# stevenlsw/reart

Measured on NVIDIA B200. Metric: skinned_chamfer_fwd_bwd_directed_point_pairs_per_s, higher is better.
Workload: dtype f32

## Files before the change

### include/reart_b200.h

```cpp
#ifndef REART_B200_H_
#define REART_B200_H_

#include <stdint.h>

#ifdef __cplusplus
extern "C" {
#endif

#if defined(__GNUC__)
#define REART_API __attribute__((visibility("default")))
#else
#define REART_API
#endif

#define REART_OK 0
#define REART_ERR_INVALID_ARG (-1)
#define REART_ERR_WORKSPACE (-2)
#define REART_ERR_LAUNCH (-3)
#define REART_ERR_UNSUPPORTED (-4)

REART_API const char* reart_version(void);
REART_API const char* reart_error_string(int code);
REART_API const char* reart_last_cuda_error(void);

// ... 42 lines not shown
REART_API int reart_skinned_chamfer_fwd_bwd_culled(const float* cano, const float* W, const float* R, const float* tr,
                                                   const float* tgt, const float* tgt_packed, int64_t T, int64_t N,
                                                   int64_t M, int64_t P, float* skinned, double* loss, float* gW,
                                                   float* gR, float* gtr, float* g_skinned, int compute_grad,
                                                   float* d_fwd, int64_t* i_fwd, float* d_bwd, int64_t* i_bwd,
                                                   int32_t* nn_rows, int32_t* nn_cols, uint64_t* cull_stats,
                                                   void* workspace, int64_t workspace_bytes, void* stream);
REART_API int reart_skinned_chamfer_fwd_bwd_ordered(const float* cano, const float* W, const float* R, const float* tr,
                                                    const float* tgt, const float* tgt_search, const float* tgt_search_packed,
                                                    int64_t T, int64_t N, int64_t M, int64_t P, const int32_t* row_order,
                                                    const int32_t* row_inv, const int32_t* tgt_order, const int32_t* tgt_inv,
                                                    float* skinned, double* loss, float* gW, float* gR, float* gtr,
                                                    float* g_skinned, int compute_grad, float* d_fwd, int64_t* i_fwd,
                                                    float* d_bwd, int64_t* i_bwd, int32_t* nn_rows, int32_t* nn_cols,
                                                    uint64_t* stats, void* workspace, int64_t workspace_bytes, void* stream);
REART_API int reart_skinned_chamfer_fwd_bwd_fused(const float* cano, const float* hot, const float* W, const float* R,
                                                  const float* tr, const float* tgt, const float* tgt_packed, int64_t T,
                                                  int64_t N, int64_t M, int64_t P, float* skinned, double* loss, float* gW,
                                                  float* gR, float* gtr, float* g_skinned, int compute_grad,
                                                  void* workspace, int64_t workspace_bytes, void* stream);


REART_API int reart_segmlp_fwd(const float* x, const float* w0, const float* b0, const float* w2, int64_t N, int64_t H,
                               int64_t P, float* logits, void* stream);
REART_API int reart_segmlp_bwd(const float* x, const float* w0, const float* b0, const float* w2, const float* glogits,
                               int64_t N, int64_t H, int64_t P, float* gw0, float* gb0, float* gw2, void* stream);
REART_API int reart_gumbel_st_fwd(const float* logits, const float* expo, const float* tau, int64_t N, int64_t P,
                                  float* W, float* ysoft, void* stream);
REART_API int reart_gumbel_st_bwd(const float* ysoft, const float* tau, const float* gW, int64_t N, int64_t P,
                                  float* glogits, void* stream);
// ... 124 lines not shown
```

### reart_b200/_lib.py

```python
from __future__ import annotations

import ctypes
import os

import torch

_HERE = os.path.dirname(os.path.abspath(__file__))
SO_PATH = os.path.join(_HERE, "csrc", "libreart_b200.so")

_c_i64 = ctypes.c_int64
_c_int = ctypes.c_int
_vp = ctypes.c_void_p

SIGNATURES = {
    "reart_version": (ctypes.c_char_p, []),
    "reart_error_string": (ctypes.c_char_p, [_c_int]),
    "reart_last_cuda_error": (ctypes.c_char_p, []),
    "reart_knn1_workspace_bytes": (_c_i64, [_c_i64, _c_i64, _c_i64]),
    "reart_knn1_fwd": (_c_int, [_vp, _vp, _c_i64, _c_i64, _c_i64, _vp, _vp, _vp, _c_i64, _vp]),
    "reart_chamfer_workspace_bytes": (_c_i64, [_c_i64, _c_i64, _c_i64]),
    "reart_chamfer_bidir_fwd": (_c_int, [_vp, _vp, _c_i64, _c_i64, _c_i64, _vp, _vp, _vp, _vp, _vp, _c_i64, _vp]),
    "reart_chamfer_sym_search": (_c_int, [_vp, _vp, _c_i64, _c_i64, _c_i64, _vp, _vp, ctypes.POINTER(ctypes.c_int32), _c_int,
                                          _vp]),
    "reart_knn1_bwd": (_c_int, [_vp, _vp, _vp, _vp, _c_i64, _c_i64, _c_i64, _vp, _vp, _vp]),
# ... 1 lines not shown
    "reart_packed_bytes": (_c_i64, [_c_i64, _c_i64]),
    "reart_pack_cloud": (_c_int, [_vp, _c_i64, _c_i64, _vp, _vp]),
    "reart_skin_fwd": (_c_int, [_vp, _vp, _vp, _vp, _c_i64, _c_i64, _c_i64, _vp, _vp]),
    "reart_skin_bwd_workspace_bytes": (_c_i64, [_c_i64, _c_i64, _c_i64]),
    "reart_skin_bwd": (_c_int, [_vp, _vp, _vp, _vp, _vp, _c_i64, _c_i64, _c_i64, _vp, _vp, _vp, _vp, _c_i64, _vp]),
    "reart_energy_workspace_bytes": (_c_i64, [_c_i64, _c_i64, _c_i64]),
    "reart_skinned_chamfer_fwd_bwd": (_c_int, [_vp, _vp, _vp, _vp, _vp, _vp, _c_i64, _c_i64, _c_i64, _c_i64, _vp, _vp,
                                               _vp, _vp, _vp, _vp, _c_int, _vp, _c_i64, _vp]),
    "reart_skinned_chamfer_fwd_bwd_ex": (_c_int, [_vp, _vp, _vp, _vp, _vp, _vp, _c_i64, _c_i64, _c_i64, _c_i64, _vp, _vp,
                                                  _vp, _vp, _vp, _vp, _c_int, _vp, _vp, _vp, _vp, _vp, _c_i64, _vp]),
    "reart_skinned_chamfer_fwd_bwd_culled": (_c_int, [_vp, _vp, _vp, _vp, _vp, _vp, _c_i64, _c_i64, _c_i64, _c_i64, _vp, _vp,
                                                      _vp, _vp, _vp, _vp, _c_int, _vp, _vp, _vp, _vp, _vp, _vp, _vp, _vp, _c_i64,
                                                      _vp]),
    "reart_skinned_chamfer_fwd_bwd_ordered": (_c_int, [_vp] * 7 + [_c_i64] * 4 + [_vp] * 10 + [_c_int] + [_vp] * 8 +
                                              [_c_i64, _vp]),
    "reart_segmlp_fwd": (_c_int, [_vp, _vp, _vp, _vp, _c_i64, _c_i64, _c_i64, _vp, _vp]),
    "reart_segmlp_bwd": (_c_int, [_vp, _vp, _vp, _vp, _vp, _c_i64, _c_i64, _c_i64, _vp, _vp, _vp, _vp]),
    "reart_gumbel_st_fwd": (_c_int, [_vp, _vp, _vp, _c_i64, _c_i64, _vp, _vp, _vp]),
    "reart_gumbel_st_bwd": (_c_int, [_vp, _vp, _vp, _c_i64, _c_i64, _vp, _vp]),
    "reart_rot6d_fwd": (_c_int, [_vp, _c_i64, _vp, _vp]),
    "reart_rot6d_bwd": (_c_int, [_vp, _vp, _c_i64, _vp, _vp]),
    "reart_screw_to_transform_fwd": (_c_int, [_vp, _vp, _vp, _vp, _c_i64, _vp, _vp]),
    "reart_screw_to_transform_bwd": (_c_int, [_vp, _vp, _vp, _vp, _vp, _c_i64, _vp, _vp, _vp, _vp, _vp]),
    "reart_fk_fwd": (_c_int, [_vp, _vp, _vp, _vp, _vp, _vp, _vp, _vp, _c_i64, _c_i64, _vp, _vp]),
    "reart_fk_bwd": (_c_int, [_vp, _vp, _vp, _vp, _vp, _vp, _vp, _vp, _c_i64, _c_i64, _vp, _vp, _vp, _vp, _vp, _vp,
                              _vp, _vp]),
    "reart_knn": (_c_int, [_vp, _vp, _c_i64, _c_i64, _c_i64, _c_int, _vp, _vp, _vp]),
    "reart_knn_sq": (_c_int, [_vp, _vp, _c_i64, _c_i64, _c_i64, _c_int, _vp, _vp, _vp]),
    "reart_knn3_blend": (_c_int, [_vp, _vp, _vp, _vp, _c_i64, _c_i64, _vp, _vp, _vp]),
    "reart_flow_refs_sorted_bytes": (_c_i64, [_c_i64, _c_i64]),
# ... 97 lines not shown
```

### reart_b200/csrc/capi.cu

```cuda
#include "../../include/reart_b200.h"
#include "common.cuh"
#include "kernels.h"

using namespace reart;

namespace {

constexpr int64_t kAlign = 256;
inline int64_t align_up(int64_t v) { return round_up(v, kAlign); }
inline bool fits_int(int64_t v) { return v >= 0 && v <= 0x7fffffff; }

#define REART_ENTRY() (void)cudaGetLastError()

struct Carver {
    char* base;
    int64_t off;
    int64_t cap;
    bool ok;
    Carver(void* p, int64_t bytes) : base(static_cast<char*>(p)), off(0), cap(bytes), ok(p != nullptr || bytes == 0) {}
    template <typename T>
    T* take(int64_t count) {
        const int64_t bytes = align_up(count * (int64_t)sizeof(T));
        if (!ok || off + bytes > cap) { ok = false; return nullptr; }
        T* r = reinterpret_cast<T*>(base + off);
// ... 205 lines not shown
                                            compute_grad, nullptr, nullptr, nullptr, nullptr, workspace, workspace_bytes, stream_);
}

int reart_skinned_chamfer_fwd_bwd_ex(const float* cano, const float* W, const float* R, const float* tr, const float* tgt,
                                     const float* tgt_packed, int64_t T, int64_t N, int64_t M, int64_t P, float* skinned,
                                     double* loss, float* gW, float* gR, float* gtr, float* g_skinned, int compute_grad,
                                     float* d_fwd, int64_t* i_fwd, float* d_bwd, int64_t* i_bwd, void* workspace,
                                     int64_t workspace_bytes, void* stream_) {
    REART_ENTRY();
    return reart_skinned_chamfer_fwd_bwd_culled(cano, W, R, tr, tgt, tgt_packed, T, N, M, P, skinned, loss, gW, gR, gtr, g_skinned,
                                                compute_grad, d_fwd, i_fwd, d_bwd, i_bwd, nullptr, nullptr, nullptr, workspace,
                                                workspace_bytes, stream_);
}

struct SearchOrder {
    const int32_t* row_order; const int32_t* row_inv; const int32_t* tgt_order; const int32_t* tgt_inv;
    const float* tgt_search;
};

static int energy_pipeline(const float* cano, const float* W, const float* hot, const float* R, const float* tr,
                           const float* tgt, const float* tgt_packed, int64_t T, int64_t N, int64_t M, int64_t P,
                           float* skinned, double* loss, float* gW, float* gR, float* gtr, float* g_skinned, int compute_grad,
                           float* d_fwd, int64_t* i_fwd, float* d_bwd, int64_t* i_bwd, int32_t* nn_rows, int32_t* nn_cols,
                           uint64_t* cull_stats, void* workspace, int64_t workspace_bytes, void* stream_,
                           const SearchOrder* order = nullptr);

int reart_skinned_chamfer_fwd_bwd_culled(const float* cano, const float* W, const float* R, const float* tr,
                                         const float* tgt, const float* tgt_packed, int64_t T, int64_t N, int64_t M,
                                         int64_t P, float* skinned, double* loss, float* gW, float* gR, float* gtr,
                                         float* g_skinned, int compute_grad, float* d_fwd, int64_t* i_fwd, float* d_bwd,
                                         int64_t* i_bwd, int32_t* nn_rows, int32_t* nn_cols, uint64_t* cull_stats,
                                         void* workspace, int64_t workspace_bytes, void* stream_) {
// ... 1 lines not shown
    return energy_pipeline(cano, W, nullptr, R, tr, tgt, tgt_packed, T, N, M, P, skinned, loss, gW, gR, gtr, g_skinned,
                           compute_grad, d_fwd, i_fwd, d_bwd, i_bwd, nn_rows, nn_cols, cull_stats, workspace, workspace_bytes,
                           stream_);
}

int reart_skinned_chamfer_fwd_bwd_ordered(const float* cano, const float* W, const float* R, const float* tr,
                                          const float* tgt, const float* tgt_search, const float* tgt_search_packed,
                                          int64_t T, int64_t N, int64_t M, int64_t P, const int32_t* row_order,
                                          const int32_t* row_inv, const int32_t* tgt_order, const int32_t* tgt_inv,
                                          float* skinned, double* loss, float* gW, float* gR, float* gtr, float* g_skinned,
                                          int compute_grad, float* d_fwd, int64_t* i_fwd, float* d_bwd, int64_t* i_bwd,
                                          int32_t* nn_rows, int32_t* nn_cols, uint64_t* stats, void* workspace,
                                          int64_t workspace_bytes, void* stream_) {
    REART_ENTRY();
    if (!tgt_search || !row_order || !row_inv || !tgt_order || !tgt_inv || !nn_rows || !nn_cols) return REART_ERR_INVALID_ARG;
    const SearchOrder order = {row_order, row_inv, tgt_order, tgt_inv, tgt_search};
    return energy_pipeline(cano, W, nullptr, R, tr, tgt, tgt_search_packed, T, N, M, P, skinned, loss, gW, gR, gtr, g_skinned,
                           compute_grad, d_fwd, i_fwd, d_bwd, i_bwd, nn_rows, nn_cols, stats, workspace, workspace_bytes,
                           stream_, &order);
}

int reart_skinned_chamfer_fwd_bwd_fused(const float* cano, const float* hot, const float* W, const float* R,
                                        const float* tr, const float* tgt, const float* tgt_packed, int64_t T, int64_t N,
                                        int64_t M, int64_t P, float* skinned, double* loss, float* gW, float* gR,
                                        float* gtr, float* g_skinned, int compute_grad, void* workspace,
                                        int64_t workspace_bytes, void* stream_) {
    REART_ENTRY();
    if (!hot || (reinterpret_cast<uintptr_t>(hot) & 15) || (reinterpret_cast<uintptr_t>(cano) & 15) ||
        (reinterpret_cast<uintptr_t>(skinned) & 15))
        return REART_ERR_INVALID_ARG;
    return energy_pipeline(cano, W, hot, R, tr, tgt, tgt_packed, T, N, M, P, skinned, loss, gW, gR, gtr, g_skinned, compute_grad,
// ... 32 lines not shown
    if (!ws.ok) return REART_ERR_WORKSPACE;
    long long* acc = reinterpret_cast<long long*>(zero);
    unsigned* ticket = reinterpret_cast<unsigned*>(zero + T * N * 24);
    unsigned* col_bound = ticket + 1;
    if (cudaMemsetAsync(zero, 0, (size_t)zero_bytes, stream) != cudaSuccess) return REART_ERR_LAUNCH;
    int rc = kOk;
    SymParams sp = {};
    sp.a = skinned; sp.b_packed = tgt_packed; sp.keys_a = ka; sp.keys_b = kb;
    sp.B = (int)T; sp.na = (int)N; sp.nb = (int)M; sp.nb_pad = (int)padded_points(M);
    sp.col_bound = col_bound;
    sp.keys_one_allocation = 1;
    if (hot) {
        if (cull) return REART_ERR_INVALID_ARG;
        sp.sk_cano = cano; sp.sk_hot = hot; sp.sk_R = R; sp.sk_tr = tr; sp.sk_P = (int)P; sp.sk_npad = (int)n_pad_sorted;
        sp.sk_out = skinned; sp.sk_sorted = psrc; sp.sk_perm = perm; sp.sk_xq = xq;
    } else {
        rc = launch_skin_fwd_sorted(cano, W, R, tr, T, N, P, skinned, psrc, perm, xq, n_pad_sorted, stream,
                                    order ? order->row_order : nullptr, skinned_search);
        if (rc) return rc;
    }
    if (order) {
        sp.a = skinned_search;
        sp.tie_a = tie; sp.tie_b = tie + T * N;
    }
    if (cull) {
        CullParams cp = {};
        cp.a = sp.a; cp.b = order ? order->tgt_search : tgt; cp.nn_rows = nn_rows; cp.nn_cols = nn_cols;
        cp.B = (int)T; cp.na = (int)N; cp.nb = (int)M; cp.nb_pad = (int)padded_points(M);
        cp.colbox = colbox; cp.rowbound = rowbound;
        cp.coarse = (N >= 8192 && M >= 8192 && N <= 800000 && M <= 800000) ? 1 : 0;
        rc = launch_cull_bounds(cp, stream);
        if (rc) return rc;
        sp.cull = 1; sp.colbox = colbox; sp.rowbound = rowbound;
        sp.cull_stats = reinterpret_cast<unsigned long long*>(cull_stats);
    }
    rc = launch_chamfer_sym(sp, stream);
    if (rc) return rc;
    EnergyParams ep = {};
    ep.src = skinned; ep.tgt = tgt; ep.src_packed = psrc; ep.tgt_packed = tgt_packed; ep.keys_a = ka; ep.keys_b = kb;
    ep.B = (int)T; ep.N = (int)N; ep.M = (int)M; ep.n_pad = (int)n_pad_sorted; ep.m_pad = (int)padded_points(M);
    ep.row_chunk_pts = kChunk; ep.col_chunk_pts = sp.col_chunk_pts; ep.gscale = 1.0f; ep.g_src = gs; ep.loss = loss;
    if (sp.col_chunk_pts != 256) return REART_ERR_UNSUPPORTED;
    ep.d_fwd = d_fwd; ep.i_fwd = i_fwd; ep.d_bwd = d_bwd; ep.i_bwd = i_bwd;
    ep.nn_rows = nn_rows; ep.nn_cols = nn_cols;
    ep.src_perm = perm; ep.src_xq = xq; ep.acc = acc; ep.col_bound = col_bound; ep.partials = partials; ep.ticket = ticket;
    if (order) {
        ep.row_order = order->row_order; ep.row_inv = order->row_inv; ep.tgt_order = order->tgt_order; ep.tgt_inv = order->tgt_inv;
        ep.tie_a = sp.tie_a; ep.tie_b = sp.tie_b;
        ep.ties = cull_stats ? reinterpret_cast<unsigned long long*>(cull_stats) + 2 : nullptr;
    }
    rc = launch_energy_bwd(ep, stream);
    if (rc || !compute_grad) return rc;
    return launch_skin_bwd(cano, W, R, tr, gs, T, N, P, gW, gR, gtr, bwd_partials, stream);
}

int reart_segmlp_fwd(const float* x, const float* w0, const float* b0, const float* w2, int64_t N, int64_t H, int64_t P,
                     float* logits, void* stream_) {
    REART_ENTRY();
    if (N < 0 || H <= 0 || P <= 0) return REART_ERR_INVALID_ARG;
    if (N == 0) return REART_OK;
    if (!x || !w0 || !b0 || !w2 || !logits) return REART_ERR_INVALID_ARG;
    return launch_segmlp(x, w0, b0, w2, nullptr, N, H, P, logits, nullptr, nullptr, nullptr,
// ... 389 lines not shown
```

### reart_b200/csrc/cull.cu

```cuda
#include "common.cuh"
#include "kernels.h"
#include <algorithm>

namespace reart {

constexpr int kCullRowChunk = 256;
constexpr int kCullSeeds = 4;
constexpr int kCoarse = 256;

__device__ __forceinline__ float coarse_upper_bound(const float* __restrict__ pts, int n, const float* __restrict__ s_rep,
                                                    int nrep, float qx, float qy, float qz) {
    float a0 = INFINITY, a1 = INFINITY;
    int r0 = 0, r1 = 0;
    for (int r = 0; r < nrep; ++r) {
        const float d = sqdist_scalar(qx, qy, qz, s_rep[3 * r], s_rep[3 * r + 1], s_rep[3 * r + 2]);
        if (d < a0) { a1 = a0; r1 = r0; a0 = d; r0 = r; }
        else if (d < a1) { a1 = d; r1 = r; }
    }
    float ub = a0;
    float b0 = INFINITY;
    int c0 = -1;
#pragma unroll 1
    for (int h = 0; h < 2; ++h) {
        const int r = h ? r1 : r0;
// ... 48 lines not shown
    }
    unsigned bits = 0u;
    if (i < p.na) {
        float ub = INFINITY;
        const float* a = p.a + ((int64_t)b * p.na + i) * 3;
        const float ax = a[0], ay = a[1], az = a[2];
        if (p.coarse) {
            ub = coarse_upper_bound(p.b + (int64_t)b * p.nb * 3, p.nb, s_rep, nrep, ax, ay, az);
            if (!(ub >= 0.f)) ub = INFINITY;
        }
        if (p.nn_rows) {
            int jprev = -2;
#pragma unroll
            for (int d = -kCullSeeds; d <= kCullSeeds; ++d) {
                const int in = min(max(i + d, 0), p.na - 1);
                const int j = p.nn_rows[(int64_t)b * p.na + in];
                if (j == jprev) continue;
                jprev = j;
                if (j >= 0 && j < p.nb) {
                    const float* t = p.b + ((int64_t)b * p.nb + j) * 3;
                    const float c = sqdist_scalar(ax, ay, az, t[0], t[1], t[2]);
                    if (c < ub) ub = c;
                }
            }
        }
        bits = __float_as_uint(ub);
    }
    bits = __reduce_max_sync(0xffffffffu, bits);
    if ((threadIdx.x & 31) == 0) s_w[threadIdx.x >> 5] = bits;
    __syncthreads();
    if (threadIdx.x == 0) {
        unsigned m = 0u;
#pragma unroll
        for (int w = 0; w < kCullRowChunk / 32; ++w) m = max(m, s_w[w]);
        p.rowbound[(int64_t)b * row_chunks + rc] = __uint_as_float(m);
// ... 15 lines not shown
    float lx = INFINITY, ly = INFINITY, lz = INFINITY, hx = -INFINITY, hy = -INFINITY, hz = -INFINITY;
    unsigned bits = 0u;
    if (j < p.nb) {
        const float* t = p.b + ((int64_t)b * p.nb + j) * 3;
        const float x = t[0], y = t[1], z = t[2];
        lx = hx = x; ly = hy = y; lz = hz = z;
        float ub = INFINITY;
        if (p.coarse) {
            ub = coarse_upper_bound(p.a + (int64_t)b * p.na * 3, p.na, s_rep, nrep, x, y, z);
            if (!(ub >= 0.f)) ub = INFINITY;
        }
        if (p.nn_cols) {
#pragma unroll
            for (int d = -kCullSeeds; d <= kCullSeeds; ++d) {
                const int jn = min(max(j + d, 0), p.nb - 1);
                const int i0 = p.nn_cols[(int64_t)b * p.nb + jn];
                if (i0 < 0 || i0 >= p.na) continue;
#pragma unroll
                for (int e = -1; e <= 1; ++e) {
                    if (d != 0 && e != 0) continue;
                    const int i = min(max(i0 + e, 0), p.na - 1);
                    const float* a = p.a + ((int64_t)b * p.na + i) * 3;
                    const float c = sqdist_scalar(a[0], a[1], a[2], x, y, z);
                    if (c < ub) ub = c;
                }
            }
        }
        bits = __float_as_uint(ub);
    }
#pragma unroll
    for (int o = 16; o > 0; o >>= 1) {
        lx = fminf(lx, __shfl_xor_sync(0xffffffffu, lx, o)); ly = fminf(ly, __shfl_xor_sync(0xffffffffu, ly, o));
// ... 29 lines not shown
```

### reart_b200/csrc/energy.cu

```cuda
#include "common.cuh"
#include "kernels.h"
#include <algorithm>

namespace reart {

constexpr int kEnergyThreads = 256;

__device__ __forceinline__ double block_sum(double local, double* sh) {
#pragma unroll
    for (int o = 16; o > 0; o >>= 1) local += __shfl_xor_sync(0xffffffffu, local, o);
    if ((threadIdx.x & 31) == 0) sh[threadIdx.x >> 5] = local;
    __syncthreads();
    double s = 0.0;
    if (threadIdx.x == 0) {
#pragma unroll
        for (int w = 0; w < kEnergyThreads / 32; ++w) s += sh[w];
    }
    return s;
}

__device__ __forceinline__ int warp_lowest_match(const float* __restrict__ pts, int n, float qx, float qy, float qz, float d) {
    const int lane = threadIdx.x & 31;
    constexpr int kPer = 16;
    for (int j0 = 0; j0 < n; j0 += 32 * kPer) {
// ... 43 lines not shown
        int i = 0;
        bool flagged = false;
        if (valid) {
            b = f / p.M;
            s = ORDERED ? b * p.M + p.tgt_inv[f] : f;
            const u64 key = p.keys_b[s];
            dmin = __uint_as_float((unsigned)(key >> 32));
            const float* a = p.tgt + f * 3;
            ax = a[0]; ay = a[1]; az = a[2];
            flagged = ORDERED && p.tie_b[s] == (unsigned)(key >> 32);
            if (!flagged) {
                i = rescan_sorted_chunk_q(p.src_packed + b * (int64_t)p.n_pad * 3, p.src_perm + b * (int64_t)p.n_pad,
                                          p.src_xq + b * (int64_t)(p.n_pad / kSortedChunk) * kQuantiles,
                                          (unsigned)(key & 0xffffffffu), ax, ay, az, dmin);
                if (i >= p.N) i = 0;
                if (ORDERED) i = p.row_order[i];
            }
        }
        if (ORDERED) resolve_flagged(flagged, p.src, p.N, ax, ay, az, dmin, b, i, p.ties);
        if (!valid) continue;
        const float* t = p.src + (b * p.N + i) * 3;
        unsigned long long* go = reinterpret_cast<unsigned long long*>(p.acc) + (b * p.N + i) * 3;
        atomicAdd(go + 0, (unsigned long long)__float2ll_rn(-g2 * (ax - t[0]) * scale));
        atomicAdd(go + 1, (unsigned long long)__float2ll_rn(-g2 * (ay - t[1]) * scale));
        atomicAdd(go + 2, (unsigned long long)__float2ll_rn(-g2 * (az - t[2]) * scale));
        local += (double)dmin;
        if (p.d_bwd) p.d_bwd[f] = dmin;
        if (p.i_bwd) p.i_bwd[f] = i;
        if (p.nn_cols) p.nn_cols[s] = ORDERED ? p.row_inv[i] : i;
    }
    const double s = block_sum(local, sh);
    if (threadIdx.x == 0) p.partials[blockIdx.x] = s;
}

template <bool ORDERED>
__global__ void __launch_bounds__(kEnergyThreads) energy_rows_kernel(const EnergyParams p, int col_blocks) {
    __shared__ double sh[kEnergyThreads / 32];
    __shared__ bool last;
    const int64_t total = (int64_t)p.B * p.N;
    const float g2 = 2.0f * p.gscale;
    const float inv = ldexpf(1.0f, -fixed_point_exponent(*p.col_bound, fabsf(g2), p.M));
    double local = 0.0;
    const int lane = threadIdx.x & 31;
    for (int64_t e0 = blockIdx.x * (int64_t)blockDim.x + (threadIdx.x - lane); e0 < total; e0 += (int64_t)gridDim.x * blockDim.x) {
        const int64_t e = e0 + lane;
        const bool valid = e < total;
        int64_t b = 0, s = 0;
        float dmin = 0.f, ax = 0.f, ay = 0.f, az = 0.f;
        int j = 0;
        bool flagged = false;
        if (valid) {
            b = e / p.N;
            s = ORDERED ? b * p.N + p.row_inv[e - b * p.N] : e;
            const u64 key = p.keys_a[s];
            dmin = __uint_as_float((unsigned)(key >> 32));
            const float* a = p.src + e * 3;
            ax = a[0]; ay = a[1]; az = a[2];
            flagged = ORDERED && p.tie_a[s] == (unsigned)(key >> 32);
            if (!flagged) {
                j = rescan_chunk32(p.tgt_packed + b * (int64_t)p.m_pad * 3, (unsigned)(key & 0xffffffffu), ax, ay, az, dmin);
                if (j >= p.M) j = 0;
                if (ORDERED) j = p.tgt_order[b * p.M + j];
            }
        }
        if (ORDERED) resolve_flagged(flagged, p.tgt, p.M, ax, ay, az, dmin, b, j, p.ties);
        if (!valid) continue;
        const long long* ac = p.acc + e * 3;
        const long long c0 = ac[0], c1 = ac[1], c2 = ac[2];
        const float* t = p.tgt + (b * p.M + j) * 3;
        p.g_src[e * 3 + 0] = g2 * (ax - t[0]) + (float)c0 * inv;
        p.g_src[e * 3 + 1] = g2 * (ay - t[1]) + (float)c1 * inv;
        p.g_src[e * 3 + 2] = g2 * (az - t[2]) + (float)c2 * inv;
        local += (double)dmin;
        if (p.d_fwd) p.d_fwd[e] = dmin;
        if (p.i_fwd) p.i_fwd[e] = j;
        if (p.nn_rows) p.nn_rows[s] = ORDERED ? p.tgt_inv[b * p.M + j] : j;
    }
    const double s = block_sum(local, sh);
    if (threadIdx.x == 0) {
        p.partials[col_blocks + blockIdx.x] = s;
        __threadfence();
        last = atomicAdd(p.ticket, 1u) == gridDim.x - 1;
    }
    __syncthreads();
    if (last) {
        __shared__ double tree[kEnergyThreads];
        __threadfence();
        const volatile double* v = p.partials;
        const int n = col_blocks + (int)gridDim.x;
        double tot = 0.0;
        for (int k = threadIdx.x; k < n; k += kEnergyThreads) tot += v[k];
// ... 41 lines not shown
```

### reart_b200/csrc/kernels.h

```cpp
#pragma once
#include <cuda_runtime.h>
#include <stdint.h>

namespace reart {

struct KnnDir {
    const float* q;
    const float* tpacked;
    unsigned long long* keys;
    float* out_dists;
    int64_t* out_idx;
    int nq;
    int nt;
    int nt_pad;
    int qblocks;
    int splits;
    int keys_preset;
    int chunk_pts;
    const unsigned char* perm;
    const float* xq;
};

struct KnnParams {
    KnnDir dir[2];
// ... 24 lines not shown
    const float* sk_cano;
    const float* sk_hot;
    const float* sk_R;
    const float* sk_tr;
    int sk_P, sk_npad;
    float* sk_out;
    float* sk_sorted;
    unsigned char* sk_perm;
    float* sk_xq;
};
struct CullParams {
    const float* a;
    const float* b;
    const int32_t* nn_rows;
    const int32_t* nn_cols;
    int B, na, nb, nb_pad;
    float* colbox;
    float* rowbound;
    int coarse;
};
int launch_cull_bounds(const CullParams& p, cudaStream_t stream);

int launch_pack_cloud(const float* pts, float* packed, int64_t B, int64_t P, cudaStream_t stream);
int launch_pack_cloud_sorted(const float* pts, float* packed, unsigned char* perm, float* xq, int64_t B, int64_t P,
                             int64_t n_pad, cudaStream_t stream);
int launch_knn1_search(KnnParams& p, cudaStream_t stream);
int launch_knn1_finalize(const KnnParams& p, cudaStream_t stream);
int launch_chamfer_sym(SymParams& p, cudaStream_t stream);

int launch_knn1_bwd(const float* p1, const float* p2, const int64_t* idx, const float* grad_dists, int64_t B,
                    int64_t P1, int64_t P2, float* grad_p1, float* grad_p2, int accumulate, cudaStream_t stream);

int launch_chamfer_bidir_bwd(const float* src, const float* tgt, const int64_t* i_fwd, const int64_t* i_bwd,
                             const float* g_fwd, const float* g_bwd, int64_t B, int64_t N, int64_t M, float* grad_src,
                             float* grad_tgt, cudaStream_t stream);

int launch_skin_fwd(const float* cano, const float* W, const float* R, const float* tr, int64_t T, int64_t N, int64_t P,
                    float* out, float* out_packed, cudaStream_t stream);
int launch_skin_fwd_sorted(const float* cano, const float* W, const float* R, const float* tr, int64_t T, int64_t N,
                           int64_t P, float* out, float* out_packed, unsigned char* perm, float* xq, int64_t n_pad,
                           cudaStream_t stream, const int32_t* order = nullptr, float* out_search = nullptr);
int64_t skin_bwd_workspace_floats(int64_t T, int64_t N, int64_t P);
int launch_skin_bwd(const float* cano, const float* W, const float* R, const float* tr, const float* g, int64_t T,
                    int64_t N, int64_t P, float* gW, float* gR, float* gtr, float* partials, cudaStream_t stream);

int launch_rot6d_fwd(const float* d6, int64_t B, float* R, cudaStream_t stream);
int launch_rot6d_bwd(const float* d6, const float* gR, int64_t B, float* gd6, cudaStream_t stream);
int launch_screw_fwd(const float* l, const float* m, const float* theta, const float* d, int64_t B, float* M,
                     cudaStream_t stream);
int launch_screw_bwd(const float* l, const float* m, const float* theta, const float* d, const float* gM, int64_t B,
                     float* gl, float* gm, float* gtheta, float* gd, cudaStream_t stream);

struct FkParams {
// ... 22 lines not shown
    const unsigned long long* keys_b;
    int B, N, M, n_pad, m_pad;
    int row_chunk_pts, col_chunk_pts;
    float gscale;
    float* g_src;
    double* loss;
    long long* acc;
    const unsigned* col_bound;
    double* partials;
    unsigned* ticket;
    int32_t* nn_rows; int32_t* nn_cols;
    float* d_fwd; int64_t* i_fwd;
    float* d_bwd; int64_t* i_bwd;
    const int32_t* row_order;
    const int32_t* row_inv;
    const int32_t* tgt_order;
    const int32_t* tgt_inv;
    const unsigned* tie_a;
    const unsigned* tie_b;
    unsigned long long* ties;
};
int energy_max_blocks();
int launch_energy_bwd(const EnergyParams& p, cudaStream_t stream);

int launch_knn(const float* ref, const float* query, int64_t B, int64_t n, int64_t m, int k, float* dist, int64_t* idx,
               int squared, cudaStream_t stream);
int64_t flow_refs_sorted_floats(int64_t total_refs, int64_t T);
int launch_flow_refs_sort(const float* ref_cat, const int64_t* ref_off, int64_t T, int64_t max_refs, float* sorted,
                          int64_t* sorted_off, cudaStream_t stream);
int launch_knn3_blend_sorted(const float* query, const float* sorted, const int64_t* sorted_off, const float* flow_cat,
// ... 133 lines not shown
```

### reart_b200/engine.py

```python
from __future__ import annotations

import ctypes
import math
from typing import Optional

import torch
import torch.nn.functional as F

from . import _lib, ops
from ._lib import check, ptr, stream_ptr
from .dist import (DistContext, GradBucket, OneShotAllReduce, flow_pairs_for_rank, flow_window_plan, halo_from_previous_rank,
                   make_small_all_reduce, shard_bounds)
from .model import BaseModel, KinematicModel


class _EngineBase:
    def __init__(self, cano: torch.Tensor, frames: torch.Tensor, ctx: Optional[DistContext], use_graph: bool, flow_ref,
                 cano_idx: int, lambda_flow: float, robust_flow: bool):
        self.ctx = ctx or DistContext()
        self.use_graph = use_graph
        self._graphs = {}
        self.iteration = 0
        if frames.shape[0] < self.ctx.world_size:
            raise ValueError(f"{frames.shape[0]} frames cannot be sharded over {self.ctx.world_size} ranks: every rank must "
                             "own at least one frame (an empty shard would skip the step's collectives)")
        lo, hi = self.ctx.frames(frames.shape[0])
        self.frame_range = (lo, hi)
        self.total_frames = int(frames.shape[0])
        self.cano = cano.float().contiguous()
        self.frames = frames[lo:hi].float().contiguous()
        self.pairs_per_step_local = 2 * (hi - lo) * self.cano.shape[0] * self.frames.shape[1]
        if flow_ref is not None and (flow_ref.T != self.total_frames or not 0 <= cano_idx <= self.total_frames):
            raise ValueError(f"the flow reference needs one set per pair of the complete sequence ({self.total_frames}) and "
                             f"0 <= cano_idx <= {self.total_frames}")
        self.flow_ref, self.cano_idx, self.lambda_flow, self.robust_flow = flow_ref, cano_idx, lambda_flow, robust_flow
        self.tau = torch.ones((), device=self.cano.device)
        self.native = self.cull = self.search_culled = False
        self.sink = self.assign = self.optimizer = self.bucket = None
        self._nat = self._ingest_src = self._cur_variant = None

    def _run_iteration(self):
        src = self._ingest_src
        if src is not None:
            cano_src, frames_src = src
            self.cano.copy_(cano_src)
            self.frames.copy_(frames_src)
            ops.pack_cloud(self.frames, out=self.frames_packed)
            if self.search_culled:
                torch.gather(self.frames, 1, self._search_gather, out=self.frames_search)
                ops.pack_cloud(self.frames_search, out=self.frames_search_packed)
        if self.native:
            return self._run_iteration_native()
# ... 148 lines not shown
        finally:
            self._ingest_src = None

    def _after_replay(self, variant):
        if variant[2]:
            self.assign.have_assignment = True

    def _setup_search(self, search: str, can_order: bool, why: str):
        if search not in ("auto", "brute", "culled"):
            raise ValueError("search must be 'auto', 'brute' or 'culled'")
        if search == "culled" and not can_order:
            raise ValueError(why)
        self.search_culled = can_order and (search == "culled" or (
            search == "auto" and min(self.cano.shape[0], self.frames.shape[1]) >= SEARCH_CULLED_MIN_POINTS))
        self.search_order_rows = self.search_order_tgt = None
        if self.search_culled:
            dev = self.cano.device
            self.search_order_rows = ops.search_order(self.cano[None], 256)[0].int()
            self.search_order_tgt = ops.search_order(self.frames, 32).int()
            self.search_inv_rows = torch.empty_like(self.search_order_rows)
            self.search_inv_rows[self.search_order_rows.long()] = torch.arange(
                self.cano.shape[0], dtype=torch.int32, device=dev)
            self.search_inv_tgt = torch.empty_like(self.search_order_tgt)
            self.search_inv_tgt.scatter_(1, self.search_order_tgt.long(), torch.arange(
                self.frames.shape[1], dtype=torch.int32, device=dev)[None].expand_as(self.search_order_tgt).contiguous())
            self._search_gather = self.search_order_tgt.long()[:, :, None].expand(-1, -1, 3)
            self.frames_search = torch.gather(self.frames, 1, self._search_gather).contiguous()
            self.frames_search_packed = ops.pack_cloud(self.frames_search)

    def _search_buffers(self, b, T, N, M):
        dev = self.cano.device
        b["nn_rows"] = torch.full((T, N), -1, dtype=torch.int32, device=dev)
        b["nn_cols"] = torch.full((T, M), -1, dtype=torch.int32, device=dev)
        b["cull_stats"] = torch.zeros(3 if self.search_culled else 2, dtype=torch.int64, device=dev)

    def _search_energy(self, L, b, W, R, tr, T, N, M, P, gW, gR, gtr, g_skinned, compute_grad):
        if self.search_culled:
            check(L.reart_skinned_chamfer_fwd_bwd_ordered(
                ptr(self.cano), ptr(W), ptr(R), ptr(tr), ptr(self.frames), ptr(self.frames_search),
                ptr(self.frames_search_packed), T, N, M, P, ptr(self.search_order_rows), ptr(self.search_inv_rows),
                ptr(self.search_order_tgt), ptr(self.search_inv_tgt), ptr(b["skinned"]), ptr(b["loss64"]), ptr(gW), ptr(gR),
                ptr(gtr), ptr(g_skinned), compute_grad, None, None, None, None, ptr(b["nn_rows"]), ptr(b["nn_cols"]),
                ptr(b["cull_stats"]), ptr(b["ws"]), b["ws_bytes"], stream_ptr()), "reart_skinned_chamfer_fwd_bwd_ordered")
        else:
            check(L.reart_skinned_chamfer_fwd_bwd(
                ptr(self.cano), ptr(W), ptr(R), ptr(tr), ptr(self.frames), ptr(self.frames_packed), T, N, M, P,
                ptr(b["skinned"]), ptr(b["loss64"]), ptr(gW), ptr(gR), ptr(gtr), ptr(g_skinned), compute_grad, ptr(b["ws"]),
                b["ws_bytes"], stream_ptr()), "reart_skinned_chamfer_fwd_bwd")

    def culling_stats(self):
        if not self.native or "cull_stats" not in self._nat:
            return None
# ... 521 lines not shown
```

Before: 13200 billion.

## Reorder skinned rows per frame by posed spatial bucketing for culled chamfer search

```diff
diff --git a/include/reart_b200.h b/include/reart_b200.h
--- a/include/reart_b200.h
+++ b/include/reart_b200.h
@@ -80,6 +80,15 @@
                                                     float* g_skinned, int compute_grad, float* d_fwd, int64_t* i_fwd,
                                                     float* d_bwd, int64_t* i_bwd, int32_t* nn_rows, int32_t* nn_cols,
                                                     uint64_t* stats, void* workspace, int64_t workspace_bytes, void* stream);
+REART_API int reart_skinned_chamfer_fwd_bwd_posed(const float* cano, const float* W, const float* R, const float* tr,
+                                                  const float* tgt, const float* tgt_search, const float* tgt_search_packed,
+                                                  int64_t T, int64_t N, int64_t M, int64_t P, const int32_t* tgt_order,
+                                                  const int32_t* tgt_inv, int32_t* row_order, int32_t* row_inv,
+                                                  float* skinned, double* loss, float* gW, float* gR, float* gtr,
+                                                  float* g_skinned, int compute_grad, float* d_fwd, int64_t* i_fwd,
+                                                  float* d_bwd, int64_t* i_bwd, int32_t* nn_rows, int32_t* nn_cols,
+                                                  uint64_t* stats, void* workspace, int64_t workspace_bytes, void* stream);
+REART_API int64_t reart_posed_order_max_points(void);
 REART_API int reart_skinned_chamfer_fwd_bwd_fused(const float* cano, const float* hot, const float* W, const float* R,
                                                   const float* tr, const float* tgt, const float* tgt_packed, int64_t T,
                                                   int64_t N, int64_t M, int64_t P, float* skinned, double* loss, float* gW,
diff --git a/reart_b200/_lib.py b/reart_b200/_lib.py
--- a/reart_b200/_lib.py
+++ b/reart_b200/_lib.py
@@ -39,6 +39,9 @@
                                                       _vp]),
     "reart_skinned_chamfer_fwd_bwd_ordered": (_c_int, [_vp] * 7 + [_c_i64] * 4 + [_vp] * 10 + [_c_int] + [_vp] * 8 +
                                               [_c_i64, _vp]),
+    "reart_skinned_chamfer_fwd_bwd_posed": (_c_int, [_vp] * 7 + [_c_i64] * 4 + [_vp] * 10 + [_c_int] + [_vp] * 8 +
+                                            [_c_i64, _vp]),
+    "reart_posed_order_max_points": (_c_i64, []),
     "reart_segmlp_fwd": (_c_int, [_vp, _vp, _vp, _vp, _c_i64, _c_i64, _c_i64, _vp, _vp]),
     "reart_segmlp_bwd": (_c_int, [_vp, _vp, _vp, _vp, _vp, _c_i64, _c_i64, _c_i64, _vp, _vp, _vp, _vp]),
     "reart_gumbel_st_fwd": (_c_int, [_vp, _vp, _vp, _c_i64, _c_i64, _vp, _vp, _vp]),
diff --git a/reart_b200/csrc/capi.cu b/reart_b200/csrc/capi.cu
--- a/reart_b200/csrc/capi.cu
+++ b/reart_b200/csrc/capi.cu
@@ -243,8 +243,10 @@
 }
 
 struct SearchOrder {
-    const int32_t* row_order; const int32_t* row_inv; const int32_t* tgt_order; const int32_t* tgt_inv;
+    int32_t* row_order; int32_t* row_inv;
+    const int32_t* tgt_order; const int32_t* tgt_inv;
     const float* tgt_search;
+    bool posed;
 };
 
 static int energy_pipeline(const float* cano, const float* W, const float* hot, const float* R, const float* tr,
@@ -276,7 +278,26 @@
                                           int64_t workspace_bytes, void* stream_) {
     REART_ENTRY();
     if (!tgt_search || !row_order || !row_inv || !tgt_order || !tgt_inv || !nn_rows || !nn_cols) return REART_ERR_INVALID_ARG;
-    const SearchOrder order = {row_order, row_inv, tgt_order, tgt_inv, tgt_search};
+    const SearchOrder order = {const_cast<int32_t*>(row_order), const_cast<int32_t*>(row_inv), tgt_order, tgt_inv, tgt_search,
+                               false};
+    return energy_pipeline(cano, W, nullptr, R, tr, tgt, tgt_search_packed, T, N, M, P, skinned, loss, gW, gR, gtr, g_skinned,
+                           compute_grad, d_fwd, i_fwd, d_bwd, i_bwd, nn_rows, nn_cols, stats, workspace, workspace_bytes,
+                           stream_, &order);
+}
+
+int64_t reart_posed_order_max_points(void) { return posed_order_max_points(); }
+
+int reart_skinned_chamfer_fwd_bwd_posed(const float* cano, const float* W, const float* R, const float* tr,
+                                        const float* tgt, const float* tgt_search, const float* tgt_search_packed, int64_t T,
+                                        int64_t N, int64_t M, int64_t P, const int32_t* tgt_order, const int32_t* tgt_inv,
+                                        int32_t* row_order, int32_t* row_inv, float* skinned, double* loss, float* gW,
+                                        float* gR, float* gtr, float* g_skinned, int compute_grad, float* d_fwd,
+                                        int64_t* i_fwd, float* d_bwd, int64_t* i_bwd, int32_t* nn_rows, int32_t* nn_cols,
+                                        uint64_t* stats, void* workspace, int64_t workspace_bytes, void* stream_) {
+    REART_ENTRY();
+    if (!tgt_search || !row_order || !row_inv || !tgt_order || !tgt_inv || !nn_rows || !nn_cols) return REART_ERR_INVALID_ARG;
+    if (N > posed_order_max_points()) return REART_ERR_UNSUPPORTED;
+    const SearchOrder order = {row_order, row_inv, tgt_order, tgt_inv, tgt_search, true};
     return energy_pipeline(cano, W, nullptr, R, tr, tgt, tgt_search_packed, T, N, M, P, skinned, loss, gW, gR, gtr, g_skinned,
                            compute_grad, d_fwd, i_fwd, d_bwd, i_bwd, nn_rows, nn_cols, stats, workspace, workspace_bytes,
                            stream_, &order);
@@ -339,6 +360,12 @@
         if (cull) return REART_ERR_INVALID_ARG;
         sp.sk_cano = cano; sp.sk_hot = hot; sp.sk_R = R; sp.sk_tr = tr; sp.sk_P = (int)P; sp.sk_npad = (int)n_pad_sorted;
         sp.sk_out = skinned; sp.sk_sorted = psrc; sp.sk_perm = perm; sp.sk_xq = xq;
+    } else if (order && order->posed) {
+        rc = launch_skin_fwd(cano, W, R, tr, T, N, P, skinned, nullptr, stream);
+        if (rc) return rc;
+        rc = launch_posed_order(skinned, T, N, n_pad_sorted, order->row_order, order->row_inv, skinned_search, psrc, perm, xq,
+                                stream);
+        if (rc) return rc;
     } else {
         rc = launch_skin_fwd_sorted(cano, W, R, tr, T, N, P, skinned, psrc, perm, xq, n_pad_sorted, stream,
                                     order ? order->row_order : nullptr, skinned_search);
@@ -351,6 +378,10 @@
     if (cull) {
         CullParams cp = {};
         cp.a = sp.a; cp.b = order ? order->tgt_search : tgt; cp.nn_rows = nn_rows; cp.nn_cols = nn_cols;
+        if (order) {
+            cp.row_order = order->row_order; cp.row_inv = order->row_inv; cp.tgt_order = order->tgt_order;
+            cp.tgt_inv = order->tgt_inv; cp.row_stride = order->posed ? N : 0;
+        }
         cp.B = (int)T; cp.na = (int)N; cp.nb = (int)M; cp.nb_pad = (int)padded_points(M);
         cp.colbox = colbox; cp.rowbound = rowbound;
         cp.coarse = (N >= 8192 && M >= 8192 && N <= 800000 && M <= 800000) ? 1 : 0;
@@ -371,6 +402,7 @@
     ep.src_perm = perm; ep.src_xq = xq; ep.acc = acc; ep.col_bound = col_bound; ep.partials = partials; ep.ticket = ticket;
     if (order) {
         ep.row_order = order->row_order; ep.row_inv = order->row_inv; ep.tgt_order = order->tgt_order; ep.tgt_inv = order->tgt_inv;
+        ep.row_stride = order->posed ? N : 0;
         ep.tie_a = sp.tie_a; ep.tie_b = sp.tie_b;
         ep.ties = cull_stats ? reinterpret_cast<unsigned long long*>(cull_stats) + 2 : nullptr;
     }
diff --git a/reart_b200/csrc/cull.cu b/reart_b200/csrc/cull.cu
--- a/reart_b200/csrc/cull.cu
+++ b/reart_b200/csrc/cull.cu
@@ -86,11 +86,13 @@
 #pragma unroll
             for (int d = -kCullSeeds; d <= kCullSeeds; ++d) {
                 const int in = min(max(i + d, 0), p.na - 1);
-                const int j = p.nn_rows[(int64_t)b * p.na + in];
+                const int cr = p.row_order ? p.row_order[(int64_t)b * p.row_stride + in] : in;
+                const int j = p.nn_rows[(int64_t)b * p.na + cr];
                 if (j == jprev) continue;
                 jprev = j;
                 if (j >= 0 && j < p.nb) {
-                    const float* t = p.b + ((int64_t)b * p.nb + j) * 3;
+                    const int js = p.tgt_inv ? p.tgt_inv[(int64_t)b * p.nb + j] : j;
+                    const float* t = p.b + ((int64_t)b * p.nb + js) * 3;
                     const float c = sqdist_scalar(ax, ay, az, t[0], t[1], t[2]);
                     if (c < ub) ub = c;
                 }
@@ -136,8 +138,10 @@
 #pragma unroll
             for (int d = -kCullSeeds; d <= kCullSeeds; ++d) {
                 const int jn = min(max(j + d, 0), p.nb - 1);
-                const int i0 = p.nn_cols[(int64_t)b * p.nb + jn];
-                if (i0 < 0 || i0 >= p.na) continue;
+                const int cj = p.tgt_order ? p.tgt_order[(int64_t)b * p.nb + jn] : jn;
+                const int ic = p.nn_cols[(int64_t)b * p.nb + cj];
+                if (ic < 0 || ic >= p.na) continue;
+                const int i0 = p.row_inv ? p.row_inv[(int64_t)b * p.row_stride + ic] : ic;
 #pragma unroll
                 for (int e = -1; e <= 1; ++e) {
                     if (d != 0 && e != 0) continue;
diff --git a/reart_b200/csrc/energy.cu b/reart_b200/csrc/energy.cu
--- a/reart_b200/csrc/energy.cu
+++ b/reart_b200/csrc/energy.cu
@@ -81,7 +81,7 @@
                                           p.src_xq + b * (int64_t)(p.n_pad / kSortedChunk) * kQuantiles,
                                           (unsigned)(key & 0xffffffffu), ax, ay, az, dmin);
                 if (i >= p.N) i = 0;
-                if (ORDERED) i = p.row_order[i];
+                if (ORDERED) i = p.row_order[b * p.row_stride + i];
             }
         }
         if (ORDERED) resolve_flagged(flagged, p.src, p.N, ax, ay, az, dmin, b, i, p.ties);
@@ -94,7 +94,7 @@
         local += (double)dmin;
         if (p.d_bwd) p.d_bwd[f] = dmin;
         if (p.i_bwd) p.i_bwd[f] = i;
-        if (p.nn_cols) p.nn_cols[s] = ORDERED ? p.row_inv[i] : i;
+        if (p.nn_cols) p.nn_cols[f] = i;
     }
     const double s = block_sum(local, sh);
     if (threadIdx.x == 0) p.partials[blockIdx.x] = s;
@@ -118,7 +118,7 @@
         bool flagged = false;
         if (valid) {
             b = e / p.N;
-            s = ORDERED ? b * p.N + p.row_inv[e - b * p.N] : e;
+            s = ORDERED ? b * p.N + p.row_inv[b * p.row_stride + e - b * p.N] : e;
             const u64 key = p.keys_a[s];
             dmin = __uint_as_float((unsigned)(key >> 32));
             const float* a = p.src + e * 3;
@@ -141,7 +141,7 @@
         local += (double)dmin;
         if (p.d_fwd) p.d_fwd[e] = dmin;
         if (p.i_fwd) p.i_fwd[e] = j;
-        if (p.nn_rows) p.nn_rows[s] = ORDERED ? p.tgt_inv[b * p.M + j] : j;
+        if (p.nn_rows) p.nn_rows[e] = j;
     }
     const double s = block_sum(local, sh);
     if (threadIdx.x == 0) {
diff --git a/reart_b200/csrc/kernels.h b/reart_b200/csrc/kernels.h
--- a/reart_b200/csrc/kernels.h
+++ b/reart_b200/csrc/kernels.h
@@ -62,6 +62,8 @@
     const float* b;
     const int32_t* nn_rows;
     const int32_t* nn_cols;
+    const int32_t* row_order; const int32_t* row_inv; const int32_t* tgt_order; const int32_t* tgt_inv;
+    int64_t row_stride;
     int B, na, nb, nb_pad;
     float* colbox;
     float* rowbound;
@@ -85,6 +87,9 @@
 
 int launch_skin_fwd(const float* cano, const float* W, const float* R, const float* tr, int64_t T, int64_t N, int64_t P,
                     float* out, float* out_packed, cudaStream_t stream);
+int posed_order_max_points();
+int launch_posed_order(const float* skinned, int64_t T, int64_t N, int64_t n_pad, int32_t* row_order, int32_t* row_inv,
+                       float* out_search, float* out_packed, unsigned char* perm, float* xq, cudaStream_t stream);
 int launch_skin_fwd_sorted(const float* cano, const float* W, const float* R, const float* tr, int64_t T, int64_t N,
                            int64_t P, float* out, float* out_packed, unsigned char* perm, float* xq, int64_t n_pad,
                            cudaStream_t stream, const int32_t* order = nullptr, float* out_search = nullptr);
@@ -137,6 +142,7 @@
     float* d_bwd; int64_t* i_bwd;
     const int32_t* row_order;
     const int32_t* row_inv;
+    int64_t row_stride;
     const int32_t* tgt_order;
     const int32_t* tgt_inv;
     const unsigned* tie_a;
diff --git a/reart_b200/csrc/order.cu b/reart_b200/csrc/order.cu
--- /dev/null
+++ b/reart_b200/csrc/order.cu
@@ -0,0 +1,203 @@
+#include "common.cuh"
+#include "kernels.h"
+
+namespace reart {
+
+constexpr int kOrderThreads = 1024;
+constexpr int kOrderBuckets = 4096;
+constexpr int kOrderMaxRows = 16384;
+__host__ __device__ constexpr int order_size(int lv) { return lv == 0 ? 2048 : lv == 1 ? 512 : 256; }
+__host__ __device__ constexpr int order_cells(int lv) { return lv == 0 ? 4096 : lv == 1 ? 512 : 128; }
+
+__device__ __forceinline__ unsigned order_cell(float x, float lo, float scale, int cells) {
+    const float v = __fmul_rn(__fsub_rn(x, lo), scale);
+    if (!(v > 0.f)) return 0u;
+    return min((unsigned)(cells - 1), __float2uint_rz(v));
+}
+
+__global__ void __launch_bounds__(kOrderThreads) posed_order_kernel(const float* __restrict__ skinned, int N, int n_pad,
+                                                                     int32_t* __restrict__ row_order,
+                                                                     int32_t* __restrict__ row_inv,
+                                                                     float* __restrict__ out_search,
+                                                                     float* __restrict__ out_packed,
+                                                                     unsigned char* __restrict__ perm,
+                                                                     float* __restrict__ xq) {
+    extern __shared__ __align__(16) unsigned char sm_raw[];
+    unsigned* slot = reinterpret_cast<unsigned*>(sm_raw);
+    unsigned* cnt = slot + kOrderMaxRows;
+    unsigned* start = cnt + kOrderBuckets;
+    unsigned char* seg = reinterpret_cast<unsigned char*>(start + kOrderBuckets);
+    __shared__ float s_ext[kOrderThreads / 32][6];
+    __shared__ float s_lo[3], s_scale[3];
+    __shared__ int s_axis[3];
+    __shared__ unsigned s_wsum[kOrderThreads / 32];
+    const int t = blockIdx.x;
+    const float* __restrict__ pts = skinned + (int64_t)t * N * 3;
+    const int lane = threadIdx.x & 31, warp = threadIdx.x >> 5;
+    float lo[3] = {INFINITY, INFINITY, INFINITY}, hi[3] = {-INFINITY, -INFINITY, -INFINITY};
+    for (int k = threadIdx.x; k < N; k += blockDim.x) {
+#pragma unroll
+        for (int a = 0; a < 3; ++a) {
+            const float v = __ldg(pts + (int64_t)k * 3 + a);
+            lo[a] = fminf(lo[a], v); hi[a] = fmaxf(hi[a], v);
+        }
+        seg[k] = 0;
+    }
+#pragma unroll
+    for (int a = 0; a < 3; ++a) {
+#pragma unroll
+        for (int o = 16; o > 0; o >>= 1) {
+            lo[a] = fminf(lo[a], __shfl_xor_sync(0xffffffffu, lo[a], o));
+            hi[a] = fmaxf(hi[a], __shfl_xor_sync(0xffffffffu, hi[a], o));
+        }
+        if (lane == 0) { s_ext[warp][a] = lo[a]; s_ext[warp][3 + a] = hi[a]; }
+    }
+    __syncthreads();
+    if (threadIdx.x == 0) {
+        float l[3], ext[3];
+#pragma unroll
+        for (int a = 0; a < 3; ++a) {
+            float h = s_ext[0][3 + a];
+            l[a] = s_ext[0][a];
+            for (int w = 1; w < kOrderThreads / 32; ++w) { l[a] = fminf(l[a], s_ext[w][a]); h = fmaxf(h, s_ext[w][3 + a]); }
+            ext[a] = __fsub_rn(h, l[a]);
+        }
+        int ax[3] = {0, 1, 2};
+        for (int u = 0; u < 2; ++u)
+            for (int v = 0; v < 2 - u; ++v)
+                if (ext[ax[v + 1]] > ext[ax[v]]) { const int s = ax[v]; ax[v] = ax[v + 1]; ax[v + 1] = s; }
+#pragma unroll
+        for (int lv = 0; lv < 3; ++lv) {
+            const float e = ext[ax[lv]];
+            s_axis[lv] = ax[lv];
+            s_lo[lv] = l[ax[lv]];
+            s_scale[lv] = (e > 0.f && e < INFINITY) ? __fdiv_rn((float)order_cells(lv), e) : 0.f;
+        }
+    }
+    __syncthreads();
+    for (int lv = 0; lv < 3; ++lv) {
+        const int axis = s_axis[lv], cells = order_cells(lv);
+        const float l = s_lo[lv], scale = s_scale[lv];
+        for (int b = threadIdx.x; b < kOrderBuckets; b += blockDim.x) cnt[b] = 0u;
+        __syncthreads();
+        for (int i = threadIdx.x; i < N; i += blockDim.x) {
+            const unsigned bkt = (unsigned)seg[i] * cells + order_cell(__ldg(pts + (int64_t)i * 3 + axis), l, scale, cells);
+            atomicAdd(cnt + bkt, 1u);
+        }
+        __syncthreads();
+        unsigned c[4], sum = 0u;
+#pragma unroll
+        for (int r = 0; r < 4; ++r) { c[r] = cnt[threadIdx.x * 4 + r]; sum += c[r]; }
+        unsigned inc = sum;
+#pragma unroll
+        for (int o = 1; o < 32; o <<= 1) {
+            const unsigned v = __shfl_up_sync(0xffffffffu, inc, o);
+            if (lane >= o) inc += v;
+        }
+        if (lane == 31) s_wsum[warp] = inc;
+        __syncthreads();
+        if (warp == 0) {
+            unsigned w = s_wsum[lane], wi = w;
+#pragma unroll
+            for (int o = 1; o < 32; o <<= 1) {
+                const unsigned v = __shfl_up_sync(0xffffffffu, wi, o);
+                if (lane >= o) wi += v;
+            }
+            s_wsum[lane] = wi - w;
+        }
+        __syncthreads();
+        unsigned run = s_wsum[warp] + inc - sum;
+#pragma unroll
+        for (int r = 0; r < 4; ++r) { start[threadIdx.x * 4 + r] = run; cnt[threadIdx.x * 4 + r] = run; run += c[r]; }
+        __syncthreads();
+        for (int i = threadIdx.x; i < N; i += blockDim.x) {
+            const unsigned bkt = (unsigned)seg[i] * cells + order_cell(__ldg(pts + (int64_t)i * 3 + axis), l, scale, cells);
+            slot[atomicAdd(cnt + bkt, 1u)] = (unsigned)i;
+        }
+        __syncthreads();
+        for (int b = threadIdx.x; b < kOrderBuckets; b += blockDim.x) {
+            const unsigned s0 = start[b], s1 = cnt[b];
+            for (unsigned u = s0 + 1; u < s1; ++u) {
+                const unsigned v = slot[u];
+                unsigned w = u;
+                while (w > s0 && slot[w - 1] > v) { slot[w] = slot[w - 1]; --w; }
+                slot[w] = v;
+            }
+        }
+        __syncthreads();
+        for (int k = threadIdx.x; k < N; k += blockDim.x) seg[slot[k]] = (unsigned char)(k / order_size(lv));
+        __syncthreads();
+    }
+    const int nblk = n_pad / kSortedChunk;
+    for (int blk = warp; blk < nblk; blk += kOrderThreads / 32) {
+        u64 key[8];
+#pragma unroll
+        for (int r = 0; r < 8; ++r) {
+            const int k = blk * kSortedChunk + lane * 8 + r;
+            key[r] = k < N ? (u64)slot[k] : ~0ull;
+        }
+        warp_bitonic_sort256(key, lane);
+#pragma unroll
+        for (int r = 0; r < 8; ++r) {
+            const int k = blk * kSortedChunk + lane * 8 + r;
+            if (k < N) slot[k] = (unsigned)key[r];
+        }
+    }
+    __syncthreads();
+    for (int k = threadIdx.x; k < N; k += blockDim.x) {
+        const int idx = (int)slot[k];
+        row_order[(int64_t)t * N + k] = idx;
+        row_inv[(int64_t)t * N + idx] = k;
+        const float* p = pts + (int64_t)idx * 3;
+        float* o = out_search + ((int64_t)t * N + k) * 3;
+        o[0] = __ldg(p); o[1] = __ldg(p + 1); o[2] = __ldg(p + 2);
+    }
+    float* sorted_b = out_packed + (int64_t)t * n_pad * 3;
+    for (int blk = warp; blk < nblk; blk += kOrderThreads / 32) {
+        u64 kx[8];
+#pragma unroll
+        for (int r = 0; r < 8; ++r) {
+            const int e = lane * 8 + r, k = blk * kSortedChunk + e;
+            const float x = k < N ? __ldg(pts + (int64_t)slot[k] * 3) : INFINITY;
+            kx[r] = ((u64)orderable_bits(x) << 32) | (u64)e;
+        }
+        warp_bitonic_sort256(kx, lane);
+        unsigned long long pm = 0ull;
+#pragma unroll
+        for (int r = 0; r < 8; ++r) {
+            const int src = (int)(kx[r] & 0xffu), pos = lane * 8 + r, k = blk * kSortedChunk + src;
+            float x = INFINITY, y = INFINITY, z = INFINITY;
+            if (k < N) {
+                const float* p = pts + (int64_t)slot[k] * 3;
+                x = __ldg(p); y = __ldg(p + 1); z = __ldg(p + 2);
+            }
+            sorted_block_store(sorted_b, blk, pos, x, y, z);
+            pm |= (unsigned long long)src << (8 * r);
+            if (r == 7 && (lane & 1)) xq[((int64_t)t * nblk + blk) * kQuantiles + (pos >> 4)] = x;
+        }
+        *reinterpret_cast<unsigned long long*>(perm + (int64_t)t * n_pad + blk * kSortedChunk + lane * 8) = pm;
+    }
+}
+
+int posed_order_max_points() { return kOrderMaxRows; }
+
+int launch_posed_order(const float* skinned, int64_t T, int64_t N, int64_t n_pad, int32_t* row_order, int32_t* row_inv,
+                       float* out_search, float* out_packed, unsigned char* perm, float* xq, cudaStream_t stream) {
+    if (T <= 0 || N <= 0) return kOk;
+    if (N > kOrderMaxRows || T > 0x7fffffff || n_pad % kSortedChunk != 0 || n_pad < N) return kErrUnsupported;
+    const size_t smem = (size_t)kOrderMaxRows * 4 + 2 * (size_t)kOrderBuckets * 4 + kOrderMaxRows;
+    static bool attr_done[64] = {};
+    int devid = -1;
+    cudaGetDevice(&devid);
+    if (devid < 0 || devid >= 64 || !attr_done[devid]) {
+        if (cudaFuncSetAttribute(posed_order_kernel, cudaFuncAttributeMaxDynamicSharedMemorySize, (int)smem) != cudaSuccess)
+            return kErrUnsupported;
+        if (devid >= 0 && devid < 64) attr_done[devid] = true;
+    }
+    posed_order_kernel<<<(unsigned)T, kOrderThreads, smem, stream>>>(skinned, (int)N, (int)n_pad, row_order, row_inv,
+                                                                     out_search, out_packed, perm, xq);
+    REART_CHECK_LAUNCH();
+    return kOk;
+}
+
+}
diff --git a/reart_b200/engine.py b/reart_b200/engine.py
--- a/reart_b200/engine.py
+++ b/reart_b200/engine.py
@@ -35,7 +35,7 @@
                              f"0 <= cano_idx <= {self.total_frames}")
         self.flow_ref, self.cano_idx, self.lambda_flow, self.robust_flow = flow_ref, cano_idx, lambda_flow, robust_flow
         self.tau = torch.ones((), device=self.cano.device)
-        self.native = self.cull = self.search_culled = False
+        self.native = self.cull = self.search_culled = self.search_posed = False
         self.sink = self.assign = self.optimizer = self.bucket = None
         self._nat = self._ingest_src = self._cur_variant = None
 
@@ -214,13 +214,15 @@
         self.search_culled = can_order and (search == "culled" or (
             search == "auto" and min(self.cano.shape[0], self.frames.shape[1]) >= SEARCH_CULLED_MIN_POINTS))
         self.search_order_rows = self.search_order_tgt = None
+        self.search_posed = self.search_culled and self.cano.shape[0] <= _lib.lib().reart_posed_order_max_points()
         if self.search_culled:
             dev = self.cano.device
-            self.search_order_rows = ops.search_order(self.cano[None], 256)[0].int()
+            if not self.search_posed:
+                self.search_order_rows = ops.search_order(self.cano[None], 256)[0].int()
+                self.search_inv_rows = torch.empty_like(self.search_order_rows)
+                self.search_inv_rows[self.search_order_rows.long()] = torch.arange(
+                    self.cano.shape[0], dtype=torch.int32, device=dev)
             self.search_order_tgt = ops.search_order(self.frames, 32).int()
-            self.search_inv_rows = torch.empty_like(self.search_order_rows)
-            self.search_inv_rows[self.search_order_rows.long()] = torch.arange(
-                self.cano.shape[0], dtype=torch.int32, device=dev)
             self.search_inv_tgt = torch.empty_like(self.search_order_tgt)
             self.search_inv_tgt.scatter_(1, self.search_order_tgt.long(), torch.arange(
                 self.frames.shape[1], dtype=torch.int32, device=dev)[None].expand_as(self.search_order_tgt).contiguous())
@@ -232,10 +234,20 @@
         dev = self.cano.device
         b["nn_rows"] = torch.full((T, N), -1, dtype=torch.int32, device=dev)
         b["nn_cols"] = torch.full((T, M), -1, dtype=torch.int32, device=dev)
+        if self.search_culled and self.search_posed:
+            b["row_order"] = torch.empty((T, N), dtype=torch.int32, device=dev)
+            b["row_inv"] = torch.empty((T, N), dtype=torch.int32, device=dev)
         b["cull_stats"] = torch.zeros(3 if self.search_culled else 2, dtype=torch.int64, device=dev)
 
     def _search_energy(self, L, b, W, R, tr, T, N, M, P, gW, gR, gtr, g_skinned, compute_grad):
-        if self.search_culled:
+        if self.search_culled and self.search_posed:
+            check(L.reart_skinned_chamfer_fwd_bwd_posed(
+                ptr(self.cano), ptr(W), ptr(R), ptr(tr), ptr(self.frames), ptr(self.frames_search),
+                ptr(self.frames_search_packed), T, N, M, P, ptr(self.search_order_tgt), ptr(self.search_inv_tgt),
+                ptr(b["row_order"]), ptr(b["row_inv"]), ptr(b["skinned"]), ptr(b["loss64"]), ptr(gW), ptr(gR), ptr(gtr),
+                ptr(g_skinned), compute_grad, None, None, None, None, ptr(b["nn_rows"]), ptr(b["nn_cols"]),
+                ptr(b["cull_stats"]), ptr(b["ws"]), b["ws_bytes"], stream_ptr()), "reart_skinned_chamfer_fwd_bwd_posed")
+        elif self.search_culled:
             check(L.reart_skinned_chamfer_fwd_bwd_ordered(
                 ptr(self.cano), ptr(W), ptr(R), ptr(tr), ptr(self.frames), ptr(self.frames_search),
                 ptr(self.frames_search_packed), T, N, M, P, ptr(self.search_order_rows), ptr(self.search_inv_rows),
```

Result: faster. 14920 billion, median of 6 (+13.0%).
